# LulinZhang/BRDF-NeRF

Hardware: AMD Instinct MI355X
Metric: train rays/sec (+ MFMA% of roofline), spsbrdf-nerf 64 samples/ray, 1/2/4/8 MI355X (higher is better)
Workload: dtype bf16; 1 GPU; BASELINE config 2: Djibouti-shaped synthetic rays, spsbrdf-nerf lambert train step (pass1 64 + guided 64 samples/ray, F=512, 8 Siren layers, PE10, ds_lambda=10), 4096 rays/GPU/step (4096 rays per global step, weak scaling); rays_per_gpu=4096, n_samples=64, guided_samples=64, parallelism=dp1, settle_steps=219

## Files before the change

brdf_nerf_amd/csrc/diag.h:

```cpp
#ifdef BN_SWITCH
BN_SWITCH(BN_PHASE_TIMING)
BN_SWITCH(BN_PHASE_TIMING_WGRAD)
BN_SWITCH(BN_CLOCK_STAMP)
BN_SWITCH(BN_CLOCK_STAMP_WGRAD)
BN_SWITCH(BN_TIMELINE)
BN_SWITCH(BN_GEMM_PRIO)
BN_SWITCH(BN_NO_NT_STASH)
BN_SWITCH(BN_NO_PINGPONG)
BN_SWITCH(BN_BWD_NO_PINGPONG)
BN_SWITCH(BN_FWD_DEPTH_TRAIN)
BN_SWITCH(BN_BWD_DEPTH)
BN_SWITCH(BN_BWD_PP_DEPTH)
BN_SWITCH(BN_BWD_D_AT)
BN_SWITCH(BN_NO_FLAT_COMPOSITE)
BN_SWITCH(SKINNY_SPLITS)
BN_SWITCH(BN_W2_BLOCKS)
BN_SWITCH(BN_FILL_NO_LDS)
BN_SWITCH(BN_DIAG_D8_IN_F32)
BN_SWITCH(BN_PROBE_NO_A)
BN_SWITCH(BN_PROBE_NO_B)
BN_SWITCH(BN_PROBE_NO_D)
BN_SWITCH(BN_PROBE_NO_RIDE)
BN_SWITCH(BN_ABLATION_BUILD)
#else
#ifndef BN_GEMM_PRIO
#define BN_GEMM_PRIO 1
#endif
#ifndef BN_FWD_DEPTH_TRAIN
#define BN_FWD_DEPTH_TRAIN 6
#endif
#ifndef BN_BWD_DEPTH
#define BN_BWD_DEPTH 2
// ... 15 lines not shown
```

brdf_nerf_amd/csrc/field_bwd.hip:

```cpp
#include "field_kernels.h"
#include "field_wgrad.h"

int bn_field_adjoint_backward(const bn_field_desc *desc, const bn_field_params *params, const void *packed, const bn_points *pts,
                              const float *d_out, void *stash, void *stream);

__device__ unsigned int g_bwd_fault;
unsigned int bn_bwd_fault_read(hipStream_t) {
  unsigned int v = 0u;
  if (hipMemcpyFromSymbol(&v, HIP_SYMBOL(g_bwd_fault), sizeof(unsigned int), 0, hipMemcpyDeviceToHost) != hipSuccess) return 0x80000000u;
  return v;
}
const unsigned int *bn_bwd_fault_ptr() {
  void *p = nullptr;
  return hipGetSymbolAddress(&p, HIP_SYMBOL(g_bwd_fault)) == hipSuccess ? (const unsigned int *)p : nullptr;
}

BN_PH_DEFINE_READER(bn_debug_phase_read_bwd)
BN_CLK_DEFINE(bn_debug_clock_read_bwd)

struct BwdArgs {
  FieldGeom g;
  bn_field_desc d;
  bn_field_params p;
  PackedLayout pl;
  StashLayout sl;
  const void *packed;
  int64_t M;
  const float *out, *d_out;
  char *stash;
  int an;
  const float *amax;
};

__device__ __forceinline__ void head_y_dy(int kind, int nout, const float *o, const float *dgo, int c, float &y, float &dy) {
  if (kind == BN_HEAD_PLAIN || kind == BN_HEAD_BETA) { y = o[c]; dy = dgo[c]; }
  else if (kind == BN_HEAD_HAPKE_THETA) { y = o[0] * (1.f / 0.52359877559829887f); dy = dgo[0] * 0.52359877559829887f; }
  else {
    const float ov = nout == 1 ? o[0] : o[c];
    const float dv = nout == 1 ? dgo[0] + dgo[1] + dgo[2] : dgo[c];
    if (kind == BN_HEAD_RPV_K) { y = (ov - 1.f) * 0.5f + 0.5f; dy = 2.f * dv; }
    else if (kind == BN_HEAD_RPV_THETA) { y = ov * 0.5f + 0.5f; dy = 2.f * dv; }
    else { y = ov; dy = dv; }
  }
}

__device__ __forceinline__ void bwd_dpre(const BwdArgs &A, int64_t gm, float (&dph)[BN_DPH], float (&dpt)[4]) {
  const FieldGeom &g = A.g;
#pragma unroll
  for (int i = 0; i < BN_DPH; ++i) dph[i] = 0.f;
#pragma unroll
  for (int i = 0; i < 4; ++i) dpt[i] = 0.f;
  if (gm >= A.M) return;
  const float *o = A.out + gm * g.C, *dgo = A.d_out + gm * g.C;
  for (int hd = 0; hd < g.n_heads; ++hd) {
    const int nout = A.d.head_out[hd], kind = A.d.head_kind[hd];
    for (int c = 0; c < nout; ++c) {
      float y, dy;
      head_y_dy(kind, nout, o + g.head_col[hd], dgo + g.head_col[hd], c, y, dy);
      dph[hd * 3 + c] = kind == BN_HEAD_BETA ? dy * -expm1f(-y) : dy * y * (1.f - y);
    }
  }
  const float sraw = ((const float *)(A.stash + A.sl.sraw))[gm];
  dpt[0] = dgo[3] * sigmoid_f(sraw);
  if (A.an) dpt[0] += ((const float *)(A.stash + A.sl.sbar))[gm];
  if (g.ch_normal_lr >= 0) {
    const float *v = (const float *)(A.stash + A.sl.nraw) + gm * 4;
    const float *dn = dgo + g.ch_normal_lr;
    const float n2 = v[0] * v[0] + v[1] * v[1] + v[2] * v[2];
    const float eps = 1.1920928955078125e-07f;
    const float inv = 1.f / sqrtf(fmaxf(n2, eps));
    const float vd = v[0] * dn[0] + v[1] * dn[1] + v[2] * dn[2];
    const float k = n2 > eps ? vd * inv * inv * inv : 0.f;
#pragma unroll
    for (int i = 0; i < 3; ++i) dpt[1 + i] = -(dn[i] * inv - v[i] * k);
  }
}

__global__ void clear_words_kernel(unsigned int *p, int n) {
  for (int i = blockIdx.x * blockDim.x + threadIdx.x; i < n; i += gridDim.x * blockDim.x) p[i] = 0u;
}

template <int WHICH> __global__ __launch_bounds__(256) void grad_amax_kernel(const BwdArgs A, float *amax) {
  const FieldGeom &g = A.g;
  float mx = 0.f;
  for (int64_t gm = (int64_t)blockIdx.x * 256 + threadIdx.x; gm < A.M; gm += (int64_t)gridDim.x * 256) {
    if (WHICH == 0) {
      float dph[BN_DPH], dpt[4];
      bwd_dpre(A, gm, dph, dpt);
#pragma unroll
      for (int i = 0; i < BN_DPH; ++i) { const float a = fabsf(dph[i]); mx = (a < 3.0e38f && a > mx) ? a : mx; }
#pragma unroll
      for (int i = 0; i < 4; ++i) { const float a = fabsf(dpt[i]); mx = (a < 3.0e38f && a > mx) ? a : mx; }
    } else {
      const float *gx = (const float *)(A.stash + A.sl.gradx) + gm * 4;
      const float *dn = A.d_out + gm * g.C + g.ch_normal_an;
      const float n2 = gx[0] * gx[0] + gx[1] * gx[1] + gx[2] * gx[2];
      const float eps = 1.1920928955078125e-07f;
      const float inv = 1.f / sqrtf(fmaxf(n2, eps));
      const float gd = gx[0] * dn[0] + gx[1] * dn[1] + gx[2] * dn[2];
// ... 20 lines not shown
  for (int64_t gm = (int64_t)blockIdx.x * 4 + wave; gm < M; gm += (int64_t)gridDim.x * 4) {
    float acc[16];
#pragma unroll
    for (int c = 0; c < 16; ++c) acc[c] = 0.f;
    const T *row = dG + gm * ldg + col0;
    for (int j = lane; j < H2; j += 64) {
      const float d = (float)row[j];
#pragma unroll
      for (int c = 0; c < 16; ++c) acc[c] += d * W[j * 16 + c];
    }
#pragma unroll
    for (int c = 0; c < 16; ++c) {
#pragma unroll
      for (int o = 32; o >= 1; o >>= 1) acc[c] += __shfl_xor(acc[c], o);
    }
    if (lane < TD) {
      float v = 0.f;
#pragma unroll
      for (int c = 0; c < 16; ++c) v = lane == c ? acc[c] : v;
      d_t[gm * TD + lane] = v * osc;
    }
  }
}

template <typename T, int MT, int NTW, bool D16>
__device__ __forceinline__ void bwd_head_dG(const BwdArgs &A, int p, T *ACT, const float *DPH, int64_t , int64_t tile) {
  typedef typename DKind<T, D16>::type DK;
  typedef typename Elem<T>::vec4 vec4;
  constexpr int BM = MT * 32;
  const FieldGeom &g = A.g;
  const int F = g.F, LDA = F + Elem<T>::kPad;
  const int tid = threadIdx.x, lane = tid & 63, wave = tid >> 6, r = lane & 31, h = lane >> 5;
  const int N = g.pass_N[p];
  const int pc0 = wave * 32 * NTW;
  if (pc0 >= N) return;
  const int hl = pc0 / g.H2, hd = 2 * p + hl;
  const int nout = A.d.head_out[hd];
  const float *w2 = A.p.head_w2[hd];
  const char *DGs = A.stash + A.sl.DG[p] + (size_t)tile * dtile_bytes<DK>(BM, F);
#pragma unroll
  for (int nt = 0; nt < NTW; ++nt) {
    f32x4 wa[2][3], wb[2][3];
#pragma unroll
    for (int gp = 0; gp < 2; ++gp) {
      const int nl = pc0 + nt * 32 + 16 * gp + 4 * h - hl * g.H2;
#pragma unroll
// ... 5 lines not shown
#pragma unroll
    for (int mt = 0; mt < MT; ++mt) {
      const int m = mt * 32 + r;
      const float d0 = DPH[m * BN_DPH + hd * 3 + 0], d1 = DPH[m * BN_DPH + hd * 3 + 1], d2 = DPH[m * BN_DPH + hd * 3 + 2];
      const DPiece<DK> pc = dpiece_load<DK>(DGs + dpiece_off<DK, MT, NTW>(wave, nt, mt, lane));
#pragma unroll
      for (int gp = 0; gp < 2; ++gp) {
        const int n0 = pc0 + nt * 32 + 16 * gp + 4 * h;
        float dg[8];
        dpiece_get<DK>(pc, gp, g.act, 1.f, dg);
        float va[4], vb[4];
#pragma unroll
        for (int e = 0; e < 4; ++e) {
          va[e] = (d0 * wa[gp][0][e] + d1 * wa[gp][1][e] + d2 * wa[gp][2][e]) * dg[e];
          vb[e] = (d0 * wb[gp][0][e] + d1 * wb[gp][1][e] + d2 * wb[gp][2][e]) * dg[4 + e];
        }
        *(vec4 *)(ACT + (size_t)m * LDA + n0) = to_vec4(T(), va[0], va[1], va[2], va[3]);
        *(vec4 *)(ACT + (size_t)m * LDA + n0 + 8) = to_vec4(T(), vb[0], vb[1], vb[2], vb[3]);
      }
    }
  }
}

template <typename T, int MT, int NT, int WAVES, bool D16>
__global__ __launch_bounds__(WAVES * 64, 2) void field_bwd_kernel(const BwdArgs A) {
  typedef typename DKind<T, D16>::type DK;
  typedef typename Elem<T>::vec4 vec4;
  constexpr int BM = MT * 32;
  extern __shared__ __attribute__((aligned(16))) char smem[];
  const FieldGeom &g = A.g;
  const int F = g.F, LDA = F + Elem<T>::kPad, KSF = F / 16;
  T *ACT = (T *)smem;
  float *DPH = (float *)(ACT + (size_t)BM * LDA);
  float *DPT = DPH + BM * BN_DPH;
  int *WR = (int *)(DPT + BM * 4), *RD = WR + 2;

  const int tid = threadIdx.x, lane = tid & 63, wave = tid >> 6, r = lane & 31, h = lane >> 5;
  const int64_t tile = blockIdx.x, m0 = tile * BM, M = A.M;
  const T *packed = (const T *)A.packed;
  constexpr int DP = (NT == 2 && WAVES == 8 && Elem<T>::kFastMath) ? (BN_BWD_PP_DEPTH | BN_GEMM_AFFINE) : BwdDepth<T>::value;
  constexpr int NPRE = std::is_same<DK, DK8>::value ? NT : 1;
  BN_PH_DECL
  BN_CLK_BEGIN

  const float gs = chain_scale(A.amax);
  if (tid < 16) WR[tid] = 0;
  if (tid < BM) {
    const int m = tid;
    const int64_t gm = m0 + m;
    float dph[BN_DPH], dpt[4];
    bwd_dpre(A, gm, dph, dpt);
    float *sh = (float *)(A.stash + A.sl.dpre_head) + gm * BN_DPH;
    float *st = (float *)(A.stash + A.sl.dpre_trunk) + gm * 4;
#pragma unroll
    for (int i = 0; i < BN_DPH; ++i) { DPH[m * BN_DPH + i] = dph[i] * gs; sh[i] = dph[i]; }
#pragma unroll
    for (int i = 0; i < 4; ++i) { DPT[m * 4 + i] = dpt[i] * gs; st[i] = dpt[i]; }
  }
  __syncthreads();
  BN_PH(0)

  const int ncol0 = wave * 32 * NT;
  const bool wave_on = ncol0 < F;
  const int n_on = F / (32 * NT) < WAVES ? F / (32 * NT) : WAVES;
  const bool ride = NT == 2 ? true : tile_copy_exact(F, n_on, WAVES);
  f32x16 acc[NT][MT];
  zero_acc<MT, NT>(acc);
  const float zr = (A.an && A.amax) ? gs / grad_scale_from(A.amax + 1, BN_GS_TARGET_ADJ) : 1.f;

  for (int p = 0; p < g.n_pass; ++p) {
    if (g.pass_heads[p] == 2) bwd_head_dG<T, MT, NT, D16>(A, p, ACT, DPH, m0, tile);
    else bwd_head_dG<T, MT, BN_SINGLE_HEAD_NTW(NT), D16>(A, p, ACT, DPH, m0, tile);
    BN_PH(1)
    __syncthreads();
    BN_PH(2)
    BN_PH(3)
    const int KSp = g.pass_N[p] / 16;
    tile_to_global<T>(ACT, LDA, (T *)(A.stash + A.sl.dG[p]) + (size_t)m0 * g.pass_N[p], g.pass_N[p], BM, g.pass_N[p]);
    if (wave_on) gemm_seg<T, MT, NT, DP>(acc, packed + A.pl.bwd_head[p] + (size_t)(ncol0 / 32) * KSp * 512, KSp, ACT, LDA, lane);
    BN_PH(4)
    __syncthreads();
    BN_PH(5)
  }
  if (wave_on && !g.fold) {
#pragma unroll
    for (int nt = 0; nt < NT; ++nt)
#pragma unroll
      for (int gq = 0; gq < 4; ++gq) {
        const int n = ncol0 + nt * 32 + 8 * gq + 4 * h;
#pragma unroll
        for (int mt = 0; mt < MT; ++mt) {
          const int m = mt * 32 + r;
          *(vec4 *)(ACT + (size_t)m * LDA + n) =
              to_vec4(T(), acc[nt][mt][4 * gq], acc[nt][mt][4 * gq + 1], acc[nt][mt][4 * gq + 2], acc[nt][mt][4 * gq + 3]);
        }
      }
  }
  BN_PH(6)
  __syncthreads();
  BN_PH(7)
  BN_PH(8)

  constexpr bool NATZ = Elem<T>::kNativeY;
#ifndef BN_BWD_NO_PINGPONG
  constexpr bool PING = NT == 2 && WAVES == 8 && Elem<T>::kFastMath;
// ... 381 lines not shown
```

brdf_nerf_amd/csrc/field_fwd.hip:

```cpp
#include "field_kernels.h"

struct FwdArgs {
  FieldGeom g;
  bn_field_desc d;
  bn_field_params p;
  PackedLayout pl;
  StashLayout sl;
  const void *packed;
  bn_points pts;
  float *out;
  char *stash;
  int sigma_only;
};

#define BN_INV_2PI 0.15915494309189535f

__device__ unsigned int g_fwd_fault;
static unsigned int *g_fault_host = nullptr;
static unsigned int g_fwd_launches = 0;
const unsigned int *bn_fwd_fault_ptr() {
  void *p = nullptr;
  return hipGetSymbolAddress(&p, HIP_SYMBOL(g_fwd_fault)) == hipSuccess ? (const unsigned int *)p : nullptr;
}

// ... 32 lines not shown
  if (g.DD > 0) {
    if (g.dir_freqs > 0) {
      for (int k = 0; k < g.dir_freqs; ++k) {
        const float f = (float)(1 << k);
#pragma unroll
        for (int c = 0; c < 3; ++c) {
          float sn, co;
          sincos_t<FAST>(f * dv[c], sn, co);
          row[6 * k + c] = (T)sn;
          row[6 * k + 3 + c] = (T)co;
        }
      }
    } else {
      for (int k = 0; k < 3; ++k) row[k] = (T)dv[k];
    }
  }
  for (int k = g.DD; k < g.KT0; ++k) row[k] = (T)0.f;
  const float *te = nullptr;
  if (g.TD > 0 && gm < A.pts.n_points && A.pts.t_embed)
    te = A.pts.t_embed + (A.pts.xyz ? gm : gm / A.pts.n_samples) * g.TD;
  for (int k = g.KT0; k < g.KD; ++k) row[k] = (T)((te && k - g.KT0 < g.TD) ? te[k - g.KT0] : 0.f);
}

template <typename T, int MT, int NTW, int WAVES, bool KEEP, bool DIR, bool HOT, bool D16>
__device__ __forceinline__ void head_pass(const FwdArgs &A, int p, const T *ACT, float *PRM, float *RED, int64_t m0, int64_t tile,
                                          const BnPhaseClock &phc_) {
  constexpr int BM = MT * 32;
  constexpr bool FAST = Elem<T>::kFastMath;
  constexpr int DP = FwdDepth<T, KEEP>::value;
  typedef typename DKind<T, D16>::type DK;
  const FieldGeom &g = A.g;
  const int F = g.F, LDA = F + Elem<T>::kPad, KSF = F / 16;
  const int tid = threadIdx.x, lane = tid & 63, wave = tid >> 6, r = lane & 31, h = lane >> 5;
  const int64_t M = A.pts.n_points;
  constexpr bool keep = KEEP;
  const int N = g.pass_N[p];
  const int pc0 = wave * 32 * NTW;
  const bool on = pc0 < N;
  for (int n = tid; n < N; n += WAVES * 64) {
    const int hn = n / g.H2, nl = n - hn * g.H2, hdn = 2 * p + hn;
    const int nout = A.d.head_out[hdn];
    PRM[n] = A.p.head_b1[hdn][nl] * act_prescale<FAST>(g.act, 1.f);
#pragma unroll
    for (int c = 0; c < 3; ++c) PRM[(1 + c) * N + n] = c < nout ? A.p.head_w2[hdn][(size_t)c * g.H2 + nl] : 0.f;
  }
  const bool dir_on = DIR && p == 0;
  T *DIRT = (T *)((char *)PRM + 8192);
  const int LDD = g.KD + Elem<T>::kPad;
  if constexpr (DIR) {
    if (dir_on && tid < BM) fill_dir_row<T>(A, m0 + tid, DIRT + (size_t)tid * LDD);
  }
  f32x16 acc[NTW][MT];
  zero_acc<MT, NTW>(acc);
  if (on) gemm_full<T, MT, NTW, DP, HOT>(acc, (const T *)A.packed + A.pl.fwd_head[p] + (size_t)(pc0 / 32) * KSF * 512, KSF, ACT, LDA, lane);
  BN_PH(9)
  __syncthreads();
  if constexpr (DIR) {
    if (dir_on) {
      const int KSD = g.KD / 16;
      if (keep) tile_to_global<T>(DIRT, LDD, (T *)(A.stash + A.sl.dirpe) + (size_t)m0 * g.KD, g.KD, BM, g.KD);
      if (on) gemm_seg<T, MT, NTW, DP>(acc, (const T *)A.packed + A.pl.fwd_dir + (size_t)(pc0 / 32) * KSD * 512, KSD, DIRT, LDD, lane);
    }
  }
  if (on) {
    T *Gs = keep ? (T *)(A.stash + A.sl.G[p]) + (size_t)tile * BM * F : nullptr;
    char *DGs = keep ? A.stash + A.sl.DG[p] + (size_t)tile * dtile_bytes<DK>(BM, F) : nullptr;
    float part[MT][3];
#pragma unroll
    for (int mt = 0; mt < MT; ++mt) part[mt][0] = part[mt][1] = part[mt][2] = 0.f;
    auto epilogue = [&](auto act_tag) {
      constexpr int ACTK = decltype(act_tag)::value;
#pragma unroll
      for (int nt = 0; nt < NTW; ++nt) {
        DHalf<DK> dh0[MT];
#pragma unroll
        for (int gp = 0; gp < 2; ++gp) {
          const int n0 = pc0 + nt * 32 + 16 * gp + 4 * h;
          const f32x4 ba = *(const f32x4 *)(PRM + n0), bb = *(const f32x4 *)(PRM + n0 + 8);
          f32x4 wa[3], wb[3];
// ... 17 lines not shown
              st_frag(Gs + native_off8<MT, NTW>(wave, nt, mt, gp, lane), yq);
              if (gp == 0) dh0[mt] = dhalf_make<DK>(dd, 1.f);
              else dpiece_store<DK>(DGs + dpiece_off<DK, MT, NTW>(wave, nt, mt, lane), dh0[mt], dhalf_make<DK>(dd, 1.f));
            }
#pragma unroll
            for (int c = 0; c < 3; ++c)
#pragma unroll
              for (int e = 0; e < 4; ++e) part[mt][c] += y[e] * wa[c][e] + y[4 + e] * wb[c][e];
          }
        }
      }
    };
    if (g.act == BN_ACT_SIN) epilogue(std::integral_constant<int, BN_ACT_SIN>());
    else epilogue(std::integral_constant<int, BN_ACT_RELU>());
#pragma unroll
    for (int mt = 0; mt < MT; ++mt)
#pragma unroll
      for (int c = 0; c < 3; ++c) {
        float v = part[mt][c];
        v += __shfl_xor(v, 32);
        if (h == 0) RED[(wave * 3 + c) * BM + mt * 32 + r] = v;
      }
  }
  BN_PH(10)
  __syncthreads();
  if (tid < BM * g.pass_heads[p]) {
    const int m = tid % BM, hl2 = tid / BM, hd2 = 2 * p + hl2;
    const int64_t gm = m0 + m;
    const int wph = g.H2 / (32 * NTW);
    const int nout = A.d.head_out[hd2], kind = A.d.head_kind[hd2];
    float v[3];
#pragma unroll
    for (int c = 0; c < 3; ++c) {
      float s = 0.f;
      for (int w = hl2 * wph; w < (hl2 + 1) * wph; ++w) s += RED[(w * 3 + c) * BM + m];
      v[c] = c < nout ? (kind == BN_HEAD_BETA ? softplus_f(s + A.p.head_b2[hd2][c]) : sigmoid_f(s + A.p.head_b2[hd2][c])) : 0.f;
    }
    if (gm < M) {
      float *o = A.out + gm * g.C + g.head_col[hd2];
      if (kind == BN_HEAD_PLAIN || kind == BN_HEAD_BETA) {
        for (int c = 0; c < nout; ++c) o[c] = v[c];
      } else if (kind == BN_HEAD_HAPKE_THETA) {
        o[0] = v[0] * 0.52359877559829887f;
      } else {
#pragma unroll
        for (int c = 0; c < 3; ++c) {
          float y = nout == 1 ? v[0] : v[c];
          if (kind == BN_HEAD_RPV_K) y = (y - 0.5f) * 2.f + 1.f;
          else if (kind == BN_HEAD_RPV_THETA) y = (y - 0.5f) * 2.f;
          o[c] = y;
        }
      }
    }
  }
  __syncthreads();
  BN_PH(11)
}

template <typename T, int MT, int NT, int WAVES, bool KEEP, bool DIR, bool D16>
__global__ __launch_bounds__(WAVES * 64, 2) void field_fwd_kernel(const FwdArgs A) {
  typedef typename Elem<T>::vec4 vec4;
  typedef typename DKind<T, D16>::type DK;
  constexpr int BM = MT * 32;
  constexpr int PADE = Elem<T>::kPad;
  constexpr bool FAST = Elem<T>::kFastMath;
  constexpr bool NATY = Elem<T>::kNativeY;
  constexpr int DP = FwdDepth<T, KEEP>::value;
  extern __shared__ __attribute__((aligned(16))) char smem[];
  const FieldGeom &g = A.g;
  const int F = g.F, LDA = F + PADE, KP = g.KP, LDP = KP + PADE;
  T *ACT = (T *)smem;
  T *PE = ACT + (size_t)BM * LDA;
  float *RED = (float *)(PE + (size_t)BM * LDP);
// ... 209 lines not shown
                *(vec4 *)(ACT + (size_t)m * LDA + n0) = to_vec4(T(), y[0], y[1], y[2], y[3]);
                *(vec4 *)(ACT + (size_t)m * LDA + n0 + 8) = to_vec4(T(), y[4], y[5], y[6], y[7]);
              }
              if (keep) {
                if (gp == 0) dh0[mt] = dhalf_make<DK>(dd, dsc);
                else dpiece_store<DK>(Ds + dpiece_off<DK, MT, NT>(wave, nt, mt, lane), dh0[mt], dhalf_make<DK>(dd, dsc));
              }
            }
          }
        }
      };
      if (g.act == BN_ACT_SIN) epilogue(std::integral_constant<int, BN_ACT_SIN>());
      else epilogue(std::integral_constant<int, BN_ACT_RELU>());
    }
    BN_PH(3)
    __syncthreads();
    BN_PH(4)
    }
  }
  if (PING) __syncthreads();
  BN_TL(9)
  BN_TL_DUMP

  if constexpr (FAST) {
    const bool nlr = g.ch_normal_lr >= 0 && !A.sigma_only;
    float *SRED = (float *)PE;
    const int nks_w = (KSF + WAVES - 1) / WAVES, ks0 = wave * nks_w;
    const bool kon = ks0 < KSF;
    const int nks = kon ? (KSF - ks0 < nks_w ? KSF - ks0 : nks_w) : 0;
    f32x16 sacc[1][MT], nacc[1][MT];
    zero_acc<MT, 1>(sacc);
    zero_acc<MT, 1>(nacc);
    if (kon) {
      if constexpr (NT == 2 && WAVES == 8) {
        gemm_fixed<T, MT, 1, 4, 4, 0>(sacc, packed + A.pl.fwd_sigma, KSF, ks0, ACT, LDA, lane, NoMid());
        if (nlr) gemm_fixed<T, MT, 1, 4, 4, 0>(nacc, packed + A.pl.fwd_nlr, KSF, ks0, ACT, LDA, lane, NoMid());
      } else {
        NoSide none;
        gemm_range<T, MT, 1, DP>(sacc, packed + A.pl.fwd_sigma, KSF, ks0, nks, ACT, LDA, lane, none);
        if (nlr) gemm_range<T, MT, 1, DP>(nacc, packed + A.pl.fwd_nlr, KSF, ks0, nks, ACT, LDA, lane, none);
      }
    }
    if (h == 0) {
#pragma unroll
      for (int mt = 0; mt < MT; ++mt)
        *(f32x4 *)(SRED + ((size_t)wave * BM + mt * 32 + r) * 4) = f32x4{sacc[0][mt][0], nacc[0][mt][0], nacc[0][mt][1], nacc[0][mt][2]};
    }
    __syncthreads();
    if (tid < BM) {
      const int m = tid;
      f32x4 sum = {0.f, 0.f, 0.f, 0.f};
      for (int w = 0; w < WAVES; ++w)
        if (w * nks_w < KSF) sum += *(const f32x4 *)(SRED + ((size_t)w * BM + m) * 4);
      const int64_t gm = m0 + m;
      const float sraw = sum[0] + A.p.sigma_b[0];
      const float sig = softplus_f(sraw);
      if (keep) ((float *)(A.stash + A.sl.sraw))[gm] = sraw;
      if (gm < M) {
        if (A.sigma_only) A.out[gm] = sig;
        else A.out[gm * g.C + 3] = sig;
      }
      if (nlr) {
        const float v0 = sum[1] + A.p.normal_b[0], v1 = sum[2] + A.p.normal_b[1], v2 = sum[3] + A.p.normal_b[2];
        if (keep) {
          float *nr = (float *)(A.stash + A.sl.nraw) + gm * 4;
          nr[0] = v0; nr[1] = v1; nr[2] = v2; nr[3] = 0.f;
        }
        if (gm < M) {
          const float inv = -1.f / sqrtf(fmaxf(v0 * v0 + v1 * v1 + v2 * v2, 1.1920928955078125e-07f));
          float *o = A.out + gm * g.C + g.ch_normal_lr;
          o[0] = v0 * inv; o[1] = v1 * inv; o[2] = v2 * inv;
        }
      }
    }
    __syncthreads();
  }
  else {
    constexpr int TPR = (WAVES * 64) / BM;
    const int m = tid / TPR, q = tid % TPR;
    const bool nlr = g.ch_normal_lr >= 0;
    float ds = 0.f, dn0 = 0.f, dn1 = 0.f, dn2 = 0.f;
    const T *row = ACT + (size_t)m * LDA;
    auto dot8 = [&](const float *w, const typename Elem<T>::frag &v) {
      const f32x4 wa = *(const f32x4 *)w, wb = *(const f32x4 *)(w + 4);
      return (float)v[0] * wa[0] + (float)v[1] * wa[1] + (float)v[2] * wa[2] + (float)v[3] * wa[3] + (float)v[4] * wb[0] +
             (float)v[5] * wb[1] + (float)v[6] * wb[2] + (float)v[7] * wb[3];
    };
#pragma unroll 4
    for (int c8 = q; c8 < F / 8; c8 += TPR) ds += dot8(A.p.sigma_w + c8 * 8, lds_frag<T>(row + c8 * 8));
    if (nlr) {
#pragma unroll 2
      for (int c8 = q; c8 < F / 8; c8 += TPR) {
        const typename Elem<T>::frag v = lds_frag<T>(row + c8 * 8);
        dn0 += dot8(A.p.normal_w + c8 * 8, v);
        dn1 += dot8(A.p.normal_w + F + c8 * 8, v);
        dn2 += dot8(A.p.normal_w + 2 * F + c8 * 8, v);
      }
    }
// ... 45 lines not shown
  BN_PH(7)
  __syncthreads();
  if (wave_on) {
#pragma unroll
    for (int nt = 0; nt < NT; ++nt)
#pragma unroll
      for (int gq = 0; gq < 4; ++gq) {
        const int n = ncol0 + nt * 32 + 8 * gq + 4 * h;
        const f32x4 b4 = *(const f32x4 *)(A.p.feats_b + n);
#pragma unroll
        for (int mt = 0; mt < MT; ++mt) {
          const int m = mt * 32 + r;
          *(vec4 *)(ACT + (size_t)m * LDA + n) = to_vec4(T(), acc[nt][mt][4 * gq + 0] + b4[0], acc[nt][mt][4 * gq + 1] + b4[1],
                                                         acc[nt][mt][4 * gq + 2] + b4[2], acc[nt][mt][4 * gq + 3] + b4[3]);
        }
      }
  }
  __syncthreads();
  if (keep) tile_to_global<T>(ACT, LDA, (T *)(A.stash + A.sl.feats) + (size_t)m0 * F, F, BM, F);
  }
  BN_PH(8)

  for (int p = 0; p < g.n_pass; ++p) {
    if (g.pass_heads[p] == 2) head_pass<T, MT, NT, WAVES, KEEP, DIR, NT == 2, D16>(A, p, ACT, (float *)PE, RED, m0, tile, phc_);
    else head_pass<T, MT, BN_SINGLE_HEAD_NTW(NT), WAVES, KEEP, DIR, NT == 2, D16>(A, p, ACT, (float *)PE, RED, m0, tile, phc_);
  }
  BN_PH_FLUSH
  BN_CLK_END
}

struct PackJob {
  const float *src;
  size_t dst;
  int ld;
  int rows, K;
  int rows_pad, K_pad;
  int row_off, col_off;
  int transposed;
  int k_lo;
  int masked;
  int K_touch;
  int row_lo;
  float scale;
};
#define BN_MAX_PACK_JOBS 48
struct PackArgs {
  PackJob job[BN_MAX_PACK_JOBS];
  int n_jobs;
// ... 229 lines not shown
```

brdf_nerf_amd/csrc/field_kernels.h:

```cpp
#pragma once
#include "field.h"
#include "instrument.h"

typedef __attribute__((ext_vector_type(4))) unsigned int u32x4;
typedef __attribute__((ext_vector_type(2))) unsigned int u32x2;
template <typename V> __device__ __forceinline__ void stash_store(V *p, const V &v) {
#ifdef BN_NO_NT_STASH
  *p = v;
#else
  __builtin_nontemporal_store(v, p);
#endif
}
template <typename V> __device__ __forceinline__ V stash_load(const V *p) {
#ifdef BN_NO_NT_STASH
  return *p;
#else
  return __builtin_nontemporal_load(p);
#endif
}

__device__ __forceinline__ auto stash_rsrc(const void *base) {
  const unsigned long long b = (unsigned long long)base;
  const unsigned int lo = __builtin_amdgcn_readfirstlane((unsigned int)b), hi = __builtin_amdgcn_readfirstlane((unsigned int)(b >> 32));
  return __builtin_amdgcn_make_buffer_rsrc((void *)(((unsigned long long)hi << 32) | lo), 0, 0x7fffffff, 0x00020000);
// ... 55 lines not shown
      lp += lstep; gp += gstep;
    }
  }
};
__host__ __device__ __forceinline__ bool tile_copy_exact(int F, int n_on, int waves) { return n_on == waves && F % 256 == 0; }

typedef __attribute__((address_space(3))) int lds_int;
__device__ __forceinline__ void pp_wait(int *flag, int target, unsigned int *fault) {
  volatile lds_int *f = (volatile lds_int *)flag;
  int spin = 0;
  for (; *f < target && spin < (1 << 24); ++spin) __builtin_amdgcn_s_sleep(1);
  if (spin >= (1 << 24) && (threadIdx.x & 63) == 0) atomicOr(fault, 1u);
  asm volatile("" ::: "memory");
}
__device__ __forceinline__ void pp_signal(int *flag, int lane) {
  asm volatile("s_waitcnt lgkmcnt(0)" ::: "memory");
  if (lane == 0) __hip_atomic_fetch_add((lds_int *)flag, 1, __ATOMIC_RELAXED, __HIP_MEMORY_SCOPE_WORKGROUP);
}

#define BN_GEMM_AFFINE 64
template <typename T, bool TRAIN_FWD> struct FwdDepth { static constexpr int value = 4; };
template <> struct FwdDepth<bf16, true> { static constexpr int value = BN_FWD_DEPTH_TRAIN | BN_GEMM_AFFINE; };
template <> struct FwdDepth<f16, true> { static constexpr int value = BN_FWD_DEPTH_TRAIN | BN_GEMM_AFFINE; };
template <typename T> struct BwdDepth { static constexpr int value = Elem<T>::kFastMath ? BN_BWD_DEPTH : 4; };

template <typename T, int MT, int NTW, int DEPTH_, typename Side>
__device__ __forceinline__ void gemm_range(f32x16 (&acc)[NTW][MT], const T *__restrict__ wp, int KS, int ks0, int nks, const T *bsrc,
                                           int ldb, int lane, Side &side) {
  constexpr int DEPTH = DEPTH_ & (BN_GEMM_AFFINE - 1);
  constexpr bool AFFINE = (DEPTH_ & BN_GEMM_AFFINE) != 0;
  typedef typename Elem<T>::frag frag;
  static_assert(DEPTH % 2 == 0, "side jobs rely on an even pipeline depth");
  const int r = lane & 31, h = lane >> 5;
  const T *wl = wp + (size_t)lane * 8;
  const T *bl = bsrc + (size_t)r * ldb + 8 * h;
  const int kend = ks0 + nks;
  frag A[DEPTH][NTW];
  auto loadA = [&](frag(&a)[NTW], int ks) {
    ks = ks < kend ? ks : kend - 1;
    {
#pragma unroll
      for (int nt = 0; nt < NTW; ++nt) {
#ifdef BN_PROBE_NO_A
        if (ks >= ks0 + DEPTH) { asm volatile("" : "+v"(a[nt])); continue; }
#endif
        a[nt] = lds_frag<T>(wl + ((size_t)nt * KS + ks) * 512);
// ... 313 lines not shown
```

profiles/phase_timing.py:

```python
import ctypes, os, subprocess, sys
ROOT = os.path.dirname(os.path.dirname(os.path.abspath(__file__)))
sys.path.insert(0, ROOT)
from brdf_nerf_amd import build as B

TIMED = ("field_fwd.hip", "field_bwd.hip", "field_wgrad.hip")


def build_timing(defines=(), tag=""):
    B.build()
    objdir = os.path.join(B.HERE, "build")
    objs = [os.path.join(objdir, os.path.basename(s) + ".o") for s in B.sources() if not s.endswith(TIMED)]
    procs = []
    for src in TIMED:
        obj = os.path.join(objdir, f"{src}.timing{tag}.o")
        objs.append(obj)
        procs.append(subprocess.Popen(B.compile_command(os.path.join(B.CSRC, src), obj, ["BN_PHASE_TIMING"] + list(defines))))
    assert all(p.wait() == 0 for p in procs)
    lib = os.path.join(objdir, f"libbn_timing{tag}.so")
    subprocess.check_call([B.HIPCC, "--offload-arch=gfx950", "-shared", "-fPIC", "-o", lib] + objs)
    return lib


if __name__ == "__main__":
    defines = [a[2:] for a in sys.argv[1:] if a.startswith("-D")]
    tag = "".join("_" + d.replace("=", "") for d in defines)
    lib = build_timing(defines, tag)
    print("variant:", defines or "default")
    if "--build-only" in sys.argv:
        sys.exit(0)
    from brdf_nerf_amd import _lib
    _lib.LIB_PATH = lib
    import torch
    import bench
    from brdf_nerf_amd import load_model
    from brdf_nerf_amd import functions as Fn
    L = _lib.lib()
    wg = "BN_PHASE_TIMING_WGRAD" in defines
    for fn in (L.bn_debug_phase_read_fwd, L.bn_debug_phase_read_bwd) + ((L.bn_debug_phase_read_wgrad,) if wg else ()):
        fn.argtypes = [ctypes.c_void_p, ctypes.c_int]
    dev = torch.device("cuda", 0)
    args = bench.make_args(4096, 64, 64, "bf16")
    torch.manual_seed(0)
    model = load_model(args).to(dev)
    spec = model.spec(False, False, False)
    packed = model.repack(spec)
    b = bench.synthetic_batch(4096, 1, dev)
    z = torch.sort(torch.rand(4096, 128, device=dev) * 2, -1)[0]
    FWD = ["pe", "gemm", "bar_gemm", "epilogue", "bar_epi", "stash", "sigma", "feats_gemm", "feats_epi+stash", "head_gemm",
           "head_epi", "head_reduce", "pp_wait_h0", "pp_wait_h1"]
    BWD = ["seed", "head_dG", "bar", "dG_stash", "head_gemm", "bar", "dfeats_epi", "bar", "dfeats_stash", "gemm", "wait_readers",
           "epilogue", "wait_writers", "tail"]
    buf = (ctypes.c_ulonglong * 17)()

    def report(tag, fn, reader, names):
        for _ in range(2):
            fn()
        torch.cuda.synchronize()
        reader(buf, 1)
        fn()
        torch.cuda.synchronize()
        reader(buf, 1)
        waves = max(1, buf[16])
        tot = sum(buf[i] for i in range(16))
        print(tag, "waves", waves, "cycles/wave", tot // waves)
        for i, n in enumerate(names):
            if n:
                print(f"   {i:2d} {n:16s} {buf[i] / waves:10.0f}  {100.0 * buf[i] / max(1, tot):5.1f} %")

    report("sigma-only (inference)", lambda: Fn.field_sigma(spec, model.named(), packed, rays=b["rays"], z=z),
           L.bn_debug_phase_read_fwd, FWD)
    n = z.numel()
    out = torch.empty(n, spec.out_channels, device=dev)
    stash = torch.empty(Fn.field_stash_bytes(spec, n), dtype=torch.uint8, device=dev)
    report("training forward (stash)", lambda: Fn.field_forward_raw(spec, model.named(), packed, out, stash, rays=b["rays"], z=z),
# ... 8 lines not shown
```

Measured before the change: 605,800 rays/s.

## Merge sigma reduction into first head pass and prefetch head dG loads in backward

In the forward kernel, the sigma reduction and the first head pass's parameter staging are folded into the first head pass's reduction barrier. This removes two block-wide syncs and splits the head epilogue across all threads, one output channel each. In the backward kernel, the first pass's head weights and dG pieces are loaded before the seed computation, and the seed work is spread across all threads by head, overlapping those loads with the seed and its barrier. Both paths raise register pressure and are gated to bf16/f16 with NT=2 and 8 waves.

New measurement: 609,300 rays/s (median of 6 runs). Within noise of the previous version (+0.6%).

```diff
diff --git a/brdf_nerf_amd/csrc/diag.h b/brdf_nerf_amd/csrc/diag.h
--- a/brdf_nerf_amd/csrc/diag.h
+++ b/brdf_nerf_amd/csrc/diag.h
@@ -8,6 +8,8 @@
 BN_SWITCH(BN_NO_NT_STASH)
 BN_SWITCH(BN_NO_PINGPONG)
 BN_SWITCH(BN_BWD_NO_PINGPONG)
+BN_SWITCH(BN_NO_HEAD_MERGE)
+BN_SWITCH(BN_BWD_NO_SEED_AHEAD)
 BN_SWITCH(BN_FWD_DEPTH_TRAIN)
 BN_SWITCH(BN_BWD_DEPTH)
 BN_SWITCH(BN_BWD_PP_DEPTH)
diff --git a/brdf_nerf_amd/csrc/field_bwd.hip b/brdf_nerf_amd/csrc/field_bwd.hip
--- a/brdf_nerf_amd/csrc/field_bwd.hip
+++ b/brdf_nerf_amd/csrc/field_bwd.hip
@@ -44,22 +44,32 @@
   }
 }
 
-__device__ __forceinline__ void bwd_dpre(const BwdArgs &A, int64_t gm, float (&dph)[BN_DPH], float (&dpt)[4]) {
+__device__ __forceinline__ void bwd_dpre_head(const BwdArgs &A, int64_t gm, int hd, float (&d3)[3]) {
   const FieldGeom &g = A.g;
-#pragma unroll
-  for (int i = 0; i < BN_DPH; ++i) dph[i] = 0.f;
+  d3[0] = d3[1] = d3[2] = 0.f;
+  if (gm >= A.M || hd >= g.n_heads) return;
+  const float *o = A.out + gm * g.C, *dgo = A.d_out + gm * g.C;
+  const int nout = A.d.head_out[hd], kind = A.d.head_kind[hd], col = g.head_col[hd];
+  float o3[3], dg3[3];
+#pragma unroll
+  for (int c = 0; c < 3; ++c) {
+    const int cc = col + c < g.C ? col + c : col;
+    o3[c] = o[cc]; dg3[c] = dgo[cc];
+  }
+#pragma unroll
+  for (int c = 0; c < 3; ++c) {
+    if (c >= nout) continue;
+    float y, dy;
+    head_y_dy(kind, nout, o3, dg3, c, y, dy);
+    d3[c] = kind == BN_HEAD_BETA ? dy * -expm1f(-y) : dy * y * (1.f - y);
+  }
+}
+__device__ __forceinline__ void bwd_dpre_trunk(const BwdArgs &A, int64_t gm, float (&dpt)[4]) {
+  const FieldGeom &g = A.g;
 #pragma unroll
   for (int i = 0; i < 4; ++i) dpt[i] = 0.f;
   if (gm >= A.M) return;
-  const float *o = A.out + gm * g.C, *dgo = A.d_out + gm * g.C;
-  for (int hd = 0; hd < g.n_heads; ++hd) {
-    const int nout = A.d.head_out[hd], kind = A.d.head_kind[hd];
-    for (int c = 0; c < nout; ++c) {
-      float y, dy;
-      head_y_dy(kind, nout, o + g.head_col[hd], dgo + g.head_col[hd], c, y, dy);
-      dph[hd * 3 + c] = kind == BN_HEAD_BETA ? dy * -expm1f(-y) : dy * y * (1.f - y);
-    }
-  }
+  const float *dgo = A.d_out + gm * g.C;
   const float sraw = ((const float *)(A.stash + A.sl.sraw))[gm];
   dpt[0] = dgo[3] * sigmoid_f(sraw);
   if (A.an) dpt[0] += ((const float *)(A.stash + A.sl.sbar))[gm];
@@ -75,6 +85,16 @@
     for (int i = 0; i < 3; ++i) dpt[1 + i] = -(dn[i] * inv - v[i] * k);
   }
 }
+__device__ __forceinline__ void bwd_dpre(const BwdArgs &A, int64_t gm, float (&dph)[BN_DPH], float (&dpt)[4]) {
+#pragma unroll
+  for (int hd = 0; hd < BN_MAX_HEADS; ++hd) {
+    float d3[3];
+    bwd_dpre_head(A, gm, hd, d3);
+#pragma unroll
+    for (int c = 0; c < 3; ++c) dph[hd * 3 + c] = d3[c];
+  }
+  bwd_dpre_trunk(A, gm, dpt);
+}
 
 __global__ void clear_words_kernel(unsigned int *p, int n) {
   for (int i = blockIdx.x * blockDim.x + threadIdx.x; i < n; i += gridDim.x * blockDim.x) p[i] = 0u;
@@ -141,6 +161,37 @@
     }
   }
 }
+
+template <typename T, int MT, int NTW, bool D16> struct HeadDGLoads {
+  typedef typename DKind<T, D16>::type DK;
+  f32x4 wa[NTW][2][3], wb[NTW][2][3];
+  DPiece<DK> pc[NTW][MT];
+  __device__ __forceinline__ void load(const BwdArgs &A, int p, int64_t tile) {
+    constexpr int BM = MT * 32;
+    const FieldGeom &g = A.g;
+    const int tid = threadIdx.x, lane = tid & 63, wave = tid >> 6, h = lane >> 5;
+    const int pc0 = wave * 32 * NTW;
+    if (pc0 >= g.pass_N[p]) return;
+    const int hl = pc0 / g.H2, hd = 2 * p + hl;
+    const int nout = A.d.head_out[hd];
+    const float *w2 = A.p.head_w2[hd];
+    const char *DGs = A.stash + A.sl.DG[p] + (size_t)tile * dtile_bytes<DK>(BM, g.F);
+#pragma unroll
+    for (int nt = 0; nt < NTW; ++nt) {
+#pragma unroll
+      for (int gp = 0; gp < 2; ++gp) {
+        const int nl = pc0 + nt * 32 + 16 * gp + 4 * h - hl * g.H2;
+#pragma unroll
+        for (int c = 0; c < 3; ++c) {
+          wa[nt][gp][c] = c < nout ? *(const f32x4 *)(w2 + (size_t)c * g.H2 + nl) : f32x4{0, 0, 0, 0};
+          wb[nt][gp][c] = c < nout ? *(const f32x4 *)(w2 + (size_t)c * g.H2 + nl + 8) : f32x4{0, 0, 0, 0};
+        }
+      }
+#pragma unroll
+      for (int mt = 0; mt < MT; ++mt) pc[nt][mt] = dpiece_load<DK>(DGs + dpiece_off<DK, MT, NTW>(wave, nt, mt, lane));
+    }
+  }
+};
 
 template <typename T, int MT, int NTW, bool D16>
 __device__ __forceinline__ void bwd_head_dG(const BwdArgs &A, int p, T *ACT, const float *DPH, int64_t , int64_t tile) {
@@ -192,6 +243,41 @@
   }
 }
 
+template <typename T, int MT, int NTW, bool D16>
+__device__ __forceinline__ void bwd_head_dG_loaded(const BwdArgs &A, int p, T *ACT, const float *DPH, const HeadDGLoads<T, MT, NTW, D16> &ld) {
+  typedef typename DKind<T, D16>::type DK;
+  typedef typename Elem<T>::vec4 vec4;
+  const FieldGeom &g = A.g;
+  const int F = g.F, LDA = F + Elem<T>::kPad;
+  const int tid = threadIdx.x, lane = tid & 63, wave = tid >> 6, r = lane & 31, h = lane >> 5;
+  const int N = g.pass_N[p];
+  const int pc0 = wave * 32 * NTW;
+  if (pc0 >= N) return;
+  const int hl = pc0 / g.H2, hd = 2 * p + hl;
+#pragma unroll
+  for (int nt = 0; nt < NTW; ++nt) {
+#pragma unroll
+    for (int mt = 0; mt < MT; ++mt) {
+      const int m = mt * 32 + r;
+      const float d0 = DPH[m * BN_DPH + hd * 3 + 0], d1 = DPH[m * BN_DPH + hd * 3 + 1], d2 = DPH[m * BN_DPH + hd * 3 + 2];
+#pragma unroll
+      for (int gp = 0; gp < 2; ++gp) {
+        const int n0 = pc0 + nt * 32 + 16 * gp + 4 * h;
+        float dg[8];
+        dpiece_get<DK>(ld.pc[nt][mt], gp, g.act, 1.f, dg);
+        float va[4], vb[4];
+#pragma unroll
+        for (int e = 0; e < 4; ++e) {
+          va[e] = (d0 * ld.wa[nt][gp][0][e] + d1 * ld.wa[nt][gp][1][e] + d2 * ld.wa[nt][gp][2][e]) * dg[e];
+          vb[e] = (d0 * ld.wb[nt][gp][0][e] + d1 * ld.wb[nt][gp][1][e] + d2 * ld.wb[nt][gp][2][e]) * dg[4 + e];
+        }
+        *(vec4 *)(ACT + (size_t)m * LDA + n0) = to_vec4(T(), va[0], va[1], va[2], va[3]);
+        *(vec4 *)(ACT + (size_t)m * LDA + n0 + 8) = to_vec4(T(), vb[0], vb[1], vb[2], vb[3]);
+      }
+    }
+  }
+}
+
 template <typename T, int MT, int NT, int WAVES, bool D16>
 __global__ __launch_bounds__(WAVES * 64, 2) void field_bwd_kernel(const BwdArgs A) {
   typedef typename DKind<T, D16>::type DK;
@@ -214,8 +300,37 @@
   BN_CLK_BEGIN
 
   const float gs = chain_scale(A.amax);
+  constexpr bool AHEAD = SeedAhead<T, NT, WAVES>::value;
+  const bool two0 = g.pass_heads[0] == 2;
+  HeadDGLoads<T, MT, NT, D16> ld2;
+  HeadDGLoads<T, MT, BN_SINGLE_HEAD_NTW(NT), D16> ld1;
+  if constexpr (AHEAD) {
+    if (two0) ld2.load(A, 0, tile);
+    else ld1.load(A, 0, tile);
+  }
   if (tid < 16) WR[tid] = 0;
-  if (tid < BM) {
+  if constexpr (AHEAD) {
+    constexpr int NQ = (WAVES * 64) / BM;
+    const int m = tid % BM, q = tid / BM;
+    const int64_t gm = m0 + m;
+    float *sh = (float *)(A.stash + A.sl.dpre_head) + gm * BN_DPH;
+    float *st = (float *)(A.stash + A.sl.dpre_trunk) + gm * 4;
+#pragma unroll
+    for (int hd0 = 0; hd0 < BN_MAX_HEADS; hd0 += NQ) {
+      const int hd = hd0 + q;
+      if (hd >= BN_MAX_HEADS) continue;
+      float d3[3];
+      bwd_dpre_head(A, gm, hd, d3);
+#pragma unroll
+      for (int c = 0; c < 3; ++c) { DPH[m * BN_DPH + hd * 3 + c] = d3[c] * gs; sh[hd * 3 + c] = d3[c]; }
+    }
+    if (q == NQ - 1) {
+      float dpt[4];
+      bwd_dpre_trunk(A, gm, dpt);
+#pragma unroll
+      for (int i = 0; i < 4; ++i) { DPT[m * 4 + i] = dpt[i] * gs; st[i] = dpt[i]; }
+    }
+  } else if (tid < BM) {
     const int m = tid;
     const int64_t gm = m0 + m;
     float dph[BN_DPH], dpt[4];
@@ -227,6 +342,7 @@
 #pragma unroll
     for (int i = 0; i < 4; ++i) { DPT[m * 4 + i] = dpt[i] * gs; st[i] = dpt[i]; }
   }
+  BN_PH(14)
   __syncthreads();
   BN_PH(0)
 
@@ -238,9 +354,7 @@
   zero_acc<MT, NT>(acc);
   const float zr = (A.an && A.amax) ? gs / grad_scale_from(A.amax + 1, BN_GS_TARGET_ADJ) : 1.f;
 
-  for (int p = 0; p < g.n_pass; ++p) {
-    if (g.pass_heads[p] == 2) bwd_head_dG<T, MT, NT, D16>(A, p, ACT, DPH, m0, tile);
-    else bwd_head_dG<T, MT, BN_SINGLE_HEAD_NTW(NT), D16>(A, p, ACT, DPH, m0, tile);
+  auto head_product = [&](int p) {
     BN_PH(1)
     __syncthreads();
     BN_PH(2)
@@ -251,6 +365,16 @@
     BN_PH(4)
     __syncthreads();
     BN_PH(5)
+  };
+  if constexpr (AHEAD) {
+    if (two0) bwd_head_dG_loaded<T, MT, NT, D16>(A, 0, ACT, DPH, ld2);
+    else bwd_head_dG_loaded<T, MT, BN_SINGLE_HEAD_NTW(NT), D16>(A, 0, ACT, DPH, ld1);
+    head_product(0);
+  }
+  for (int p = AHEAD ? 1 : 0; p < g.n_pass; ++p) {
+    if (g.pass_heads[p] == 2) bwd_head_dG<T, MT, NT, D16>(A, p, ACT, DPH, m0, tile);
+    else bwd_head_dG<T, MT, BN_SINGLE_HEAD_NTW(NT), D16>(A, p, ACT, DPH, m0, tile);
+    head_product(p);
   }
   if (wave_on && !g.fold) {
 #pragma unroll
diff --git a/brdf_nerf_amd/csrc/field_fwd.hip b/brdf_nerf_amd/csrc/field_fwd.hip
--- a/brdf_nerf_amd/csrc/field_fwd.hip
+++ b/brdf_nerf_amd/csrc/field_fwd.hip
@@ -78,9 +78,9 @@
   for (int k = g.KT0; k < g.KD; ++k) row[k] = (T)((te && k - g.KT0 < g.TD) ? te[k - g.KT0] : 0.f);
 }
 
-template <typename T, int MT, int NTW, int WAVES, bool KEEP, bool DIR, bool HOT, bool D16>
+template <typename T, int MT, int NTW, int WAVES, bool KEEP, bool DIR, bool HOT, bool D16, bool RED4>
 __device__ __forceinline__ void head_pass(const FwdArgs &A, int p, const T *ACT, float *PRM, float *RED, int64_t m0, int64_t tile,
-                                          const BnPhaseClock &phc_) {
+                                          const BnPhaseClock &phc_, bool staged = false, const float *SRED = nullptr) {
   constexpr int BM = MT * 32;
   constexpr bool FAST = Elem<T>::kFastMath;
   constexpr int DP = FwdDepth<T, KEEP>::value;
@@ -93,7 +93,7 @@
   const int N = g.pass_N[p];
   const int pc0 = wave * 32 * NTW;
   const bool on = pc0 < N;
-  for (int n = tid; n < N; n += WAVES * 64) {
+  for (int n = tid; n < N && !(RED4 && staged); n += WAVES * 64) {
     const int hn = n / g.H2, nl = n - hn * g.H2, hdn = 2 * p + hn;
     const int nout = A.d.head_out[hdn];
     PRM[n] = A.p.head_b1[hdn][nl] * act_prescale<FAST>(g.act, 1.f);
@@ -110,7 +110,7 @@
   zero_acc<MT, NTW>(acc);
   if (on) gemm_full<T, MT, NTW, DP, HOT>(acc, (const T *)A.packed + A.pl.fwd_head[p] + (size_t)(pc0 / 32) * KSF * 512, KSF, ACT, LDA, lane);
   BN_PH(9)
-  __syncthreads();
+  if (!(RED4 && staged)) __syncthreads();
   if constexpr (DIR) {
     if (dir_on) {
       const int KSD = g.KD / 16;
@@ -174,33 +174,89 @@
         if (h == 0) RED[(wave * 3 + c) * BM + mt * 32 + r] = v;
       }
   }
-  BN_PH(10)
-  __syncthreads();
-  if (tid < BM * g.pass_heads[p]) {
-    const int m = tid % BM, hl2 = tid / BM, hd2 = 2 * p + hl2;
+  if constexpr (RED4) {
+    constexpr int NQ = (WAVES * 64) / BM;
+    const int m = tid % BM, q = __builtin_amdgcn_readfirstlane(tid / BM);
     const int64_t gm = m0 + m;
-    const int wph = g.H2 / (32 * NTW);
-    const int nout = A.d.head_out[hd2], kind = A.d.head_kind[hd2];
-    float v[3];
-#pragma unroll
-    for (int c = 0; c < 3; ++c) {
-      float s = 0.f;
-      for (int w = hl2 * wph; w < (hl2 + 1) * wph; ++w) s += RED[(w * 3 + c) * BM + m];
-      v[c] = c < nout ? (kind == BN_HEAD_BETA ? softplus_f(s + A.p.head_b2[hd2][c]) : sigmoid_f(s + A.p.head_b2[hd2][c])) : 0.f;
-    }
-    if (gm < M) {
-      float *o = A.out + gm * g.C + g.head_col[hd2];
-      if (kind == BN_HEAD_PLAIN || kind == BN_HEAD_BETA) {
-        for (int c = 0; c < nout; ++c) o[c] = v[c];
-      } else if (kind == BN_HEAD_HAPKE_THETA) {
-        o[0] = v[0] * 0.52359877559829887f;
-      } else {
-#pragma unroll
-        for (int c = 0; c < 3; ++c) {
-          float y = nout == 1 ? v[0] : v[c];
-          if (kind == BN_HEAD_RPV_K) y = (y - 0.5f) * 2.f + 1.f;
-          else if (kind == BN_HEAD_RPV_THETA) y = (y - 0.5f) * 2.f;
-          o[c] = y;
+    const int nhead = 3 * g.pass_heads[p], ntask = nhead + (SRED ? 1 : 0);
+    float bias[2] = {0.f, 0.f};
+#pragma unroll
+    for (int i = 0; i < 2; ++i) {
+      const int t = q + NQ * i;
+      if (t < nhead) {
+        const int hd2 = 2 * p + t / 3, c = t % 3;
+        bias[i] = A.p.head_b2[hd2][A.d.head_out[hd2] == 1 ? 0 : c];
+      } else if (t < ntask) {
+        bias[i] = A.p.sigma_b[0];
+      }
+    }
+    BN_PH(10)
+    __syncthreads();
+    BN_PH(13)
+#pragma unroll
+    for (int i = 0; i < 2; ++i) {
+      const int t = q + NQ * i;
+      if (t < nhead) {
+        const int hl2 = t / 3, c = t % 3, hd2 = 2 * p + hl2;
+        const int wph = g.H2 / (32 * NTW);
+        const int nout = A.d.head_out[hd2], kind = A.d.head_kind[hd2];
+        const int cs = nout == 1 ? 0 : c;
+        float s = 0.f;
+        for (int w = hl2 * wph; w < (hl2 + 1) * wph; ++w) s += RED[(w * 3 + cs) * BM + m];
+        const float v = kind == BN_HEAD_BETA ? softplus_f(s + bias[i]) : sigmoid_f(s + bias[i]);
+        if (gm < M) {
+          float *o = A.out + gm * g.C + g.head_col[hd2];
+          if (kind == BN_HEAD_PLAIN || kind == BN_HEAD_BETA) {
+            if (c < nout) o[c] = v;
+          } else if (kind == BN_HEAD_HAPKE_THETA) {
+            if (c == 0) o[0] = v * 0.52359877559829887f;
+          } else {
+            float y = v;
+            if (kind == BN_HEAD_RPV_K) y = (y - 0.5f) * 2.f + 1.f;
+            else if (kind == BN_HEAD_RPV_THETA) y = (y - 0.5f) * 2.f;
+            o[c] = y;
+          }
+        }
+      } else if (t < ntask) {
+        float sum = 0.f;
+        for (int w = 0; w < WAVES; ++w) sum += SRED[(size_t)w * BM + m];
+        const float sraw = sum + bias[i];
+        const float sig = softplus_f(sraw);
+        if (KEEP) ((float *)(A.stash + A.sl.sraw))[gm] = sraw;
+        if (gm < M) A.out[gm * g.C + 3] = sig;
+      }
+    }
+    if (p + 1 == g.n_pass) { BN_PH(11) return; }
+  } else {
+    BN_PH(10)
+    __syncthreads();
+    BN_PH(13)
+    if (tid < BM * g.pass_heads[p]) {
+      const int m = tid % BM, hl2 = tid / BM, hd2 = 2 * p + hl2;
+      const int64_t gm = m0 + m;
+      const int wph = g.H2 / (32 * NTW);
+      const int nout = A.d.head_out[hd2], kind = A.d.head_kind[hd2];
+      float v[3];
+#pragma unroll
+      for (int c = 0; c < 3; ++c) {
+        float s = 0.f;
+        for (int w = hl2 * wph; w < (hl2 + 1) * wph; ++w) s += RED[(w * 3 + c) * BM + m];
+        v[c] = c < nout ? (kind == BN_HEAD_BETA ? softplus_f(s + A.p.head_b2[hd2][c]) : sigmoid_f(s + A.p.head_b2[hd2][c])) : 0.f;
+      }
+      if (gm < M) {
+        float *o = A.out + gm * g.C + g.head_col[hd2];
+        if (kind == BN_HEAD_PLAIN || kind == BN_HEAD_BETA) {
+          for (int c = 0; c < nout; ++c) o[c] = v[c];
+        } else if (kind == BN_HEAD_HAPKE_THETA) {
+          o[0] = v[0] * 0.52359877559829887f;
+        } else {
+#pragma unroll
+          for (int c = 0; c < 3; ++c) {
+            float y = nout == 1 ? v[0] : v[c];
+            if (kind == BN_HEAD_RPV_K) y = (y - 0.5f) * 2.f + 1.f;
+            else if (kind == BN_HEAD_RPV_THETA) y = (y - 0.5f) * 2.f;
+            o[c] = y;
+          }
         }
       }
     }
@@ -456,6 +512,12 @@
   BN_TL(9)
   BN_TL_DUMP
 
+  constexpr bool MERGE = HeadMerge<T, NT, WAVES, KEEP, DIR>::value && PING;
+  const int N0 = g.pass_N[0];
+  const bool merge = MERGE && g.ch_normal_lr < 0 && !A.sigma_only &&
+                     (size_t)WAVES * BM * 4 + (size_t)16 * N0 <= (size_t)BM * LDP * sizeof(T) && N0 <= WAVES * 64;
+  float *SRED1 = (float *)PE, *PRM0 = SRED1 + WAVES * BM;
+
   if constexpr (FAST) {
     const bool nlr = g.ch_normal_lr >= 0 && !A.sigma_only;
     float *SRED = (float *)PE;
@@ -465,6 +527,15 @@
     f32x16 sacc[1][MT], nacc[1][MT];
     zero_acc<MT, 1>(sacc);
     zero_acc<MT, 1>(nacc);
+    const int pcol = wave * 32 * g.pass_NTW[0] + lane;
+    const bool stage = MERGE && merge && lane < 32 * g.pass_NTW[0] && pcol < N0;
+    float prm[4] = {0.f, 0.f, 0.f, 0.f};
+    if (stage) {
+      const int hn = pcol / g.H2, nl = pcol - hn * g.H2, nout = A.d.head_out[hn];
+      prm[0] = A.p.head_b1[hn][nl];
+#pragma unroll
+      for (int c = 0; c < 3; ++c) prm[1 + c] = c < nout ? A.p.head_w2[hn][(size_t)c * g.H2 + nl] : 0.f;
+    }
     if (kon) {
       if constexpr (NT == 2 && WAVES == 8) {
         gemm_fixed<T, MT, 1, 4, 4, 0>(sacc, packed + A.pl.fwd_sigma, KSF, ks0, ACT, LDA, lane, NoMid());
@@ -475,12 +546,27 @@
         if (nlr) gemm_range<T, MT, 1, DP>(nacc, packed + A.pl.fwd_nlr, KSF, ks0, nks, ACT, LDA, lane, none);
       }
     }
+    if (MERGE && merge) {
+      if (h == 0) {
+#pragma unroll
+        for (int mt = 0; mt < MT; ++mt) SRED1[(size_t)wave * BM + mt * 32 + r] = sacc[0][mt][0];
+      }
+      if (stage) {
+        PRM0[pcol] = prm[0] * act_prescale<FAST>(g.act, 1.f);
+#pragma unroll
+        for (int c = 0; c < 3; ++c) PRM0[(1 + c) * N0 + pcol] = prm[1 + c];
+      }
+      __builtin_amdgcn_wave_barrier();
+      BN_PH(14)
+    } else {
     if (h == 0) {
 #pragma unroll
       for (int mt = 0; mt < MT; ++mt)
         *(f32x4 *)(SRED + ((size_t)wave * BM + mt * 32 + r) * 4) = f32x4{sacc[0][mt][0], nacc[0][mt][0], nacc[0][mt][1], nacc[0][mt][2]};
     }
+    BN_PH(14)
     __syncthreads();
+    BN_PH(15)
     if (tid < BM) {
       const int m = tid;
       f32x4 sum = {0.f, 0.f, 0.f, 0.f};
@@ -508,6 +594,7 @@
       }
     }
     __syncthreads();
+    }
   }
   else {
     constexpr int TPR = (WAVES * 64) / BM;
@@ -599,8 +686,11 @@
   BN_PH(8)
 
   for (int p = 0; p < g.n_pass; ++p) {
-    if (g.pass_heads[p] == 2) head_pass<T, MT, NT, WAVES, KEEP, DIR, NT == 2, D16>(A, p, ACT, (float *)PE, RED, m0, tile, phc_);
-    else head_pass<T, MT, BN_SINGLE_HEAD_NTW(NT), WAVES, KEEP, DIR, NT == 2, D16>(A, p, ACT, (float *)PE, RED, m0, tile, phc_);
+    const bool first = MERGE && merge && p == 0;
+    float *PRM = first ? PRM0 : (float *)PE;
+    const float *SRED = first ? SRED1 : nullptr;
+    if (g.pass_heads[p] == 2) head_pass<T, MT, NT, WAVES, KEEP, DIR, NT == 2, D16, MERGE>(A, p, ACT, PRM, RED, m0, tile, phc_, first, SRED);
+    else head_pass<T, MT, BN_SINGLE_HEAD_NTW(NT), WAVES, KEEP, DIR, NT == 2, D16, MERGE>(A, p, ACT, PRM, RED, m0, tile, phc_, first, SRED);
   }
   BN_PH_FLUSH
   BN_CLK_END
diff --git a/brdf_nerf_amd/csrc/field_kernels.h b/brdf_nerf_amd/csrc/field_kernels.h
--- a/brdf_nerf_amd/csrc/field_kernels.h
+++ b/brdf_nerf_amd/csrc/field_kernels.h
@@ -101,6 +101,20 @@
 template <typename T, bool TRAIN_FWD> struct FwdDepth { static constexpr int value = 4; };
 template <> struct FwdDepth<bf16, true> { static constexpr int value = BN_FWD_DEPTH_TRAIN | BN_GEMM_AFFINE; };
 template <> struct FwdDepth<f16, true> { static constexpr int value = BN_FWD_DEPTH_TRAIN | BN_GEMM_AFFINE; };
+template <typename T, int NT, int WAVES> struct SeedAhead {
+#ifndef BN_BWD_NO_SEED_AHEAD
+  static constexpr bool value = sizeof(T) == 2 && NT == 2 && WAVES == 8;
+#else
+  static constexpr bool value = false;
+#endif
+};
+template <typename T, int NT, int WAVES, bool KEEP, bool DIR> struct HeadMerge {
+#ifndef BN_NO_HEAD_MERGE
+  static constexpr bool value = sizeof(T) == 2 && NT == 2 && WAVES == 8 && KEEP && !DIR;
+#else
+  static constexpr bool value = false;
+#endif
+};
 template <typename T> struct BwdDepth { static constexpr int value = Elem<T>::kFastMath ? BN_BWD_DEPTH : 4; };
 
 template <typename T, int MT, int NTW, int DEPTH_, typename Side>
diff --git a/profiles/phase_timing.py b/profiles/phase_timing.py
--- a/profiles/phase_timing.py
+++ b/profiles/phase_timing.py
@@ -24,7 +24,7 @@
 if __name__ == "__main__":
     defines = [a[2:] for a in sys.argv[1:] if a.startswith("-D")]
     tag = "".join("_" + d.replace("=", "") for d in defines)
-    lib = build_timing(defines, tag)
+    lib = os.path.join(B.HERE, "build", f"libbn_timing{tag}.so") if "--prebuilt" in sys.argv else build_timing(defines, tag)
     print("variant:", defines or "default")
     if "--build-only" in sys.argv:
         sys.exit(0)
@@ -47,9 +47,10 @@
     b = bench.synthetic_batch(4096, 1, dev)
     z = torch.sort(torch.rand(4096, 128, device=dev) * 2, -1)[0]
     FWD = ["pe", "gemm", "bar_gemm", "epilogue", "bar_epi", "stash", "sigma", "feats_gemm", "feats_epi+stash", "head_gemm",
-           "head_epi", "head_reduce", "pp_wait_h0", "pp_wait_h1"]
+           "head_epi", "head_reduce", "pp_wait_h0", "head_red_bar", "sigma_mfma",
+           "sigma_bar"]
     BWD = ["seed", "head_dG", "bar", "dG_stash", "head_gemm", "bar", "dfeats_epi", "bar", "dfeats_stash", "gemm", "wait_readers",
-           "epilogue", "wait_writers", "tail"]
+           "epilogue", "wait_writers", "tail", "seed_work"]
     buf = (ctypes.c_ulonglong * 17)()
 
     def report(tag, fn, reader, names):
```
